# VatsalPandey0202/PointCloudRegistration

Measured on AMD Instinct MI355X. Metric: TOF/PC pairs/sec (8192 pts), higher is better.
Workload: dtype f32 xyz/features; f64 RANSAC/ICP; 1-term f16 MFMA screen (certified bound), f16x3-split MFMA screen for the rows it leaves, f64 exact re-rank; 1 GPU; C4: batch of augmented TOF/PC pairs (featNN+RANSAC+ICP+Chamfer); pairs_total=256, pairs_per_gpu=256, points=8192, feature_dim=32, streams_per_gpu=1, ransac=d=0.04 mutual n=3 edge0.9 dist0.04 (100000,0.999), icp=d=0.02 (1e-6,1e-6,30), parallelism=pair-sharded x1, inputs=resident in HBM (--full: host_resident is the PCIe-inclusive rate)

## Files before the change

pointcloudregistration_amd/csrc/featnn_thresh.h:

```cpp
#pragma once
#include <stdint.h>
#include <string.h>

#if defined(__HIPCC__)
#define PCR_THRESH_HD __host__ __device__
#else
#define PCR_THRESH_HD
#endif

namespace pcr {

PCR_THRESH_HD inline uint32_t thresh_bits_up(double t) {
    if (!(t == t)) return 0x7f800000u;
    if (!(t > 0.0)) return 0u;
    const float f = (float)t;
    uint32_t b;
    memcpy(&b, &f, sizeof(b));
    return (double)f < t ? b + 1u : b;
}

PCR_THRESH_HD inline int thresh_flush_count(uint32_t base, uint32_t local, int K) {
    if (base >= (uint32_t)K) return 0;
    const uint32_t room = (uint32_t)K - base;
    return (int)(local < room ? local : room);
}

}
```

pointcloudregistration_amd/csrc/featnn_thresh.hip:

```cpp
#include "featnn_v5.h"
#include "featnn_thresh.h"
#include <stdlib.h>
#include <algorithm>
#include <cstdio>
#include <type_traits>

namespace pcr {
namespace {

__device__ unsigned g_thresh_stat[2][3];

#ifndef PCR_THRESH_G
#define PCR_THRESH_G 16
#endif
#ifndef PCR_THRESH_PF
#define PCR_THRESH_PF 1
#endif
constexpr int kThreshG = PCR_THRESH_G;

__device__ __forceinline__ unsigned lds_add_rtn(unsigned addr, unsigned v) {
    unsigned r;
    asm volatile("ds_add_rtn_u32 %0, %1, %2\n\ts_waitcnt lgkmcnt(0)" : "=v"(r) : "v"(addr), "v"(v) : "memory");
    return r;
}
__device__ __forceinline__ void lds_store(unsigned addr, int v) {
    asm volatile("ds_write_b32 %0, %1\n\ts_waitcnt lgkmcnt(0)" : : "v"(addr), "v"(v) : "memory");
}

template <int S, bool kIdx>
__global__ __launch_bounds__(512) void featnn_thresh9(RowArgs5 a) {
    constexpr int NB = S, W = 8, RT = 2, G = kThreshG, GS = G / 2;
    constexpr int kT = G * NB * 64;
    constexpr int kRows = W * RT * 32;
    static_assert(G % 2 == 0 && kRows == 512, "whole steps; the flush is one row per thread");
    __shared__ __attribute__((aligned(16))) f16x8 Bs0[kT];
    __shared__ __attribute__((aligned(16))) f16x8 Bs1[kT];
    __shared__ __attribute__((aligned(16))) float Cs0[G * 32];
    __shared__ __attribute__((aligned(16))) float Cs1[G * 32];
    __shared__ unsigned hcnt[kRows];
    __shared__ int hslot[kRows * kThreshK];
    const int nbp = gridDim.x / (8 * ((a.P + 7) >> 3));
    const int bid = blockIdx.x, xcd = bid & 7, slot = bid >> 3;
    const int p = (slot / nbp) * 8 + xcd, sl = slot % nbp;
    if (p >= a.P) return;
    const int nr = min(a.rcount[p], a.Rmax);
    const int m = count_of(a.n_cols, p, a.Cmax);
    const int nst = (((m + 31) >> 5) + 1) >> 1;
    const int nsl = min(nbp, nst);
    if (nr <= 0 || sl >= nsl) return;
    const int s0 = (int)((long long)nst * sl / nsl), s1 = (int)((long long)nst * (sl + 1) / nsl);
    const int ngr = (s1 - s0 + GS - 1) / GS;
    const int wid = threadIdx.x >> 6, l = threadIdx.x & 63, h = l >> 5;
    const int ntl = (nr + 31) >> 5;
    const int *rl = a.rlist + (size_t)p * a.Rmax;
    const int nm = a.ich;
    const f16x8 *bimg = a.Bp + (size_t)p * a.ntc * nm * 64 + l;
    const float *ctp = a.cct + (size_t)p * a.ntc * 32 + l;
    auto issue = [&](auto bufc_, int grp) {
        f16x8 *Bs = decltype(bufc_)::value ? Bs1 : Bs0;
        float *Cs = decltype(bufc_)::value ? Cs1 : Cs0;
        const int sg = s0 + grp * GS;
        for (int c = wid; c < G * NB + GS; c += W) {
            if (c >= G * NB) {
                const int j = c - G * NB;
                if (sg + j < s1)
                    __builtin_amdgcn_global_load_lds(
                        (const __attribute__((address_space(1))) void *)(ctp + (size_t)(sg + j) * 64),
                        (__attribute__((address_space(3))) void *)(Cs + j * 64),
                        4, 0, 0);
                continue;
            }
            const int g = c / NB, cc = c - g * NB;
            if (sg + (g >> 1) < s1)
                __builtin_amdgcn_global_load_lds(
                    (const __attribute__((address_space(1))) void *)(bimg + ((size_t)(2 * sg + g) * nm + cc) * 64),
                    (__attribute__((address_space(3))) void *)(Bs + c * 64), 16, 0, 0);
        }
    };
    auto min8 = [](const f32x16 &x, int q) {
        unsigned c = umin2(umin2(fbits(x[8 * q]), fbits(x[8 * q + 1])), fbits(x[8 * q + 2]));
        c = umin2(umin2(c, fbits(x[8 * q + 3])), fbits(x[8 * q + 4]));
        c = umin2(umin2(c, fbits(x[8 * q + 5])), fbits(x[8 * q + 6]));
        return umin2(c, fbits(x[8 * q + 7]));
    };
    for (int tb = 0; tb < ntl; tb += W * RT) {
        hcnt[threadIdx.x] = 0u;
        issue(std::integral_constant<int, 0>{}, 0);
        const int nt = tb + wid + W < ntl ? 2 : (tb + wid < ntl ? 1 : 0);
        size_t o[RT];
        unsigned B1[RT], thr[RT], am[RT];
        bool live[RT];
        int nh[RT], lr[RT];
        unsigned ca[RT], sa[RT];
        f16x8 A[RT][NB];
#pragma unroll
        for (int t = 0; t < RT; ++t) {
            lr[t] = (t * W + wid) * 32 + (l & 31);
            ca[t] = (unsigned)(uintptr_t)(hcnt + lr[t]);
            sa[t] = (unsigned)(uintptr_t)(hslot + lr[t] * kThreshK);
            const int k = tb * 32 + lr[t];
            const bool valid = k < nr;
            const int row = valid ? rl[k] : 0;
            o[t] = (size_t)p * a.Rmax + row;
            B1[t] = valid ? a.rec[o[t]].y : 0x7f800000u;
            thr[t] = 0u;
            live[t] = false;
            if (valid && B1[t] < 0x7f800000u) {
                const double bnd = row_bound_ct(a, p, row, a.rre[(size_t)p * a.ntr * 32 + row], 16 * S);
                thr[t] = thresh_bits_up((double)__uint_as_float(B1[t]) + bnd * (1.0 + 0x1p-20));
                live[t] = thr[t] < 0x7f800000u;
            }
            row_operand<S, 3>(a, p, row, valid, h, A[t]);
            am[t] = 0xffffffffu;
            nh[t] = 0;
        }
        auto sweep = [&](auto ntc_, auto bufc_, int grp) {
            constexpr int NT = decltype(ntc_)::value;
            const f16x8 *Bs = decltype(bufc_)::value ? Bs1 : Bs0;
            const float *Cb = decltype(bufc_)::value ? Cs1 : Cs0;
            const int sg = s0 + grp * GS, ns = min(GS, s1 - sg);
            const f16x8 *Bb = Bs + l;
            auto load = [&](int j, f16x8 (&Bf)[2][NB], f32x16 (&Cf)[2]) {
#pragma unroll
                for (int u = 0; u < 2; ++u) {
#pragma unroll
                    for (int c = 0; c < NB; ++c) Bf[u][c] = Bb[((2 * j + u) * NB + c) * 64];
                    Cf[u] = colterms(Cb + (2 * j + u) * 32, h);
                }
            };
            f16x8 Bf[2][NB];
            f32x16 Cf[2];
            if (PCR_THRESH_PF) load(0, Bf, Cf);
            for (int j = 0; j < ns; ++j) {
                const int st = sg + j;
                f16x8 Bn[2][NB];
                f32x16 Cn[2];
                if (PCR_THRESH_PF) load(j + 1 < ns ? j + 1 : j, Bn, Cn);
                else load(j, Bf, Cf);
                f32x16 acc[NT][2];
#pragma unroll
                for (int c = 0; c < NB; ++c)
#pragma unroll
                    for (int u = 0; u < 2; ++u)
#pragma unroll
                        for (int t = 0; t < NT; ++t)
                            acc[t][u] = __builtin_amdgcn_mfma_f32_32x32x16_f16(Bf[u][c], A[t][c],
                                                                               c == 0 ? Cf[u] : acc[t][u], 0, 0, 0);
#pragma unroll
                for (int t = 0; t < NT; ++t)
#pragma unroll
                    for (int u = 0; u < 2; ++u) {
                        const unsigned m0 = min8(acc[t][u], 0), m1 = min8(acc[t][u], 1);
                        if (__ballot(umin2(m0, m1) <= thr[t]) == 0ull) continue;
                        const bool half[2] = {__ballot(m0 <= thr[t]) != 0ull, __ballot(m1 <= thr[t]) != 0ull};
#pragma unroll
                        for (int r = 0; r < 16; ++r) {
                            if (!half[r >> 3]) continue;
                            const unsigned v = fbits(acc[t][u][r]);
                            const int col = 32 * (2 * st + u) + 8 * (r >> 2) + 4 * h + (r & 3);
                            if (v <= thr[t] && live[t] && col < m) {
                                if (kIdx && v == B1[t]) am[t] = umin2(am[t], (unsigned)col);
                                if (nh[t] <= kThreshK) {
                                    const unsigned pos = lds_add_rtn(ca[t], 1u);
                                    if (pos < (unsigned)kThreshK) lds_store(sa[t] + 4u * pos, col);
                                }
                                ++nh[t];
                            }
                        }
                    }
                if (PCR_THRESH_PF) {
#pragma unroll
                    for (int u = 0; u < 2; ++u) {
#pragma unroll
                        for (int c = 0; c < NB; ++c) Bf[u][c] = Bn[u][c];
                        Cf[u] = Cn[u];
                    }
                }
            }
        };
        asm volatile("s_waitcnt vmcnt(0)" ::: "memory");
        __syncthreads();
        auto group = [&](auto bufc_, int grp) {
            constexpr int buf = decltype(bufc_)::value;
            if (grp + 1 < ngr) issue(std::integral_constant<int, buf ^ 1>{}, grp + 1);
            if (nt == 2) sweep(std::integral_constant<int, 2>{}, bufc_, grp);
            else if (nt == 1) sweep(std::integral_constant<int, 1>{}, bufc_, grp);
            asm volatile("s_waitcnt vmcnt(0)" ::: "memory");
            __syncthreads();
        };
        for (int grp = 0; grp < ngr; grp += 2) {
            group(std::integral_constant<int, 0>{}, grp);
            if (grp + 1 < ngr) group(std::integral_constant<int, 1>{}, grp + 1);
        }
#pragma unroll
        for (int t = 0; t < RT; ++t)
            if (kIdx && am[t] != 0xffffffffu) atomicMin(reinterpret_cast<unsigned *>(a.rec + o[t]) + 2, am[t]);
        {
            const int r = threadIdx.x, k = tb * 32 + r;
            const unsigned lc = hcnt[r];
            if (k < nr && lc != 0u) {
                const size_t oo = (size_t)p * a.Rmax + rl[k];
                const unsigned base = atomicAdd(reinterpret_cast<unsigned *>(a.rec + oo), lc);
                const int n = thresh_flush_count(base, lc, kThreshK);
                for (int i = 0; i < n; ++i) a.cand[oo * kThreshK + base + i] = hslot[r * kThreshK + i];
            }
        }
        __syncthreads();
    }
}

template <int DV, bool kIdx>
__global__ __launch_bounds__(256) void featnn_exact_cand(RowArgs5 a) {
    const int p = blockIdx.y;
    const int nr = min(a.rcount[p], a.Rmax);
    if (nr <= 0) return;
    if (blockIdx.x == 0 && threadIdx.x == 0) atomicAdd(a.fbctr + (kIdx ? 0 : 1), (unsigned long long)nr);
    const int m = count_of(a.n_cols, p, a.Cmax);
    const int *rl = a.rlist + (size_t)p * a.Rmax;
    const int c = threadIdx.x & 7, rr = threadIdx.x >> 3, D = a.D;
    const float4 open = make_float4(__builtin_inff(), __builtin_inff(), __builtin_inff(), 0.0f);
    for (int k0 = blockIdx.x * 32; k0 < nr; k0 += gridDim.x * 32) {
        const bool act = k0 + rr < nr;
        const int row = act ? rl[k0 + rr] : 0;
        const size_t o = (size_t)p * a.Rmax + row;
        const uint4 rc = act ? a.rec[o] : make_uint4(0u, 0x7f800000u, 0u, 1u);
        const int cnt = (int)min(rc.x, (unsigned)kThreshK + 1u);
        double best = __builtin_inf();
        int bj = 0x7fffffff;
        if (act && m > 0 && c < cnt && cnt <= kThreshK && rc.y < 0x7f800000u) {
            const int j = a.cand[o * kThreshK + c];
            const float *q = a.Xr + o * D, *y = a.Xc + ((size_t)p * a.Cmax + j) * D;
            float qf[DV], yf[DV];
            if (D == DV && (((uintptr_t)q | (uintptr_t)y) & 15) == 0) {
#pragma unroll
                for (int k = 0; k < DV; k += 4) {
                    const float4 u = *reinterpret_cast<const float4 *>(q + k), w = *reinterpret_cast<const float4 *>(y + k);
                    qf[k] = u.x; qf[k + 1] = u.y; qf[k + 2] = u.z; qf[k + 3] = u.w;
                    yf[k] = w.x; yf[k + 1] = w.y; yf[k + 2] = w.z; yf[k + 3] = w.w;
                }
            } else {
#pragma unroll
                for (int k = 0; k < DV; ++k) {
                    qf[k] = k < D ? q[k] : 0.0f;
                    yf[k] = k < D ? y[k] : 0.0f;
                }
            }
            double acc = 0.0;
#pragma unroll
            for (int k = 0; k < DV; ++k) {
                const double df = (double)qf[k] - (double)yf[k];
                acc = acc + df * df;
            }
            if (acc < best) { best = acc; bj = j; }
        }
#pragma unroll
        for (int x = 1; x < 8; x <<= 1) {
            const double ob = __shfl_xor(best, x, 64);
// ... 86 lines not shown
```

pointcloudregistration_amd/csrc/featnn_row.hip:

```cpp
#include "featnn_v5.h"
#include <stdlib.h>
#include <algorithm>

namespace pcr {
namespace {

__device__ unsigned long long g_featnn_fallback_rows[2];

template <int S>
__device__ __forceinline__ void row_frags(const float *x, int D, int h, int role, int cs,
                                          f16x8 (&out)[2 * S + 1]) {
    constexpr int DV = 16 * S;
    double acc = 0.0;
#pragma unroll
    for (int k = 0; k < DV; ++k)
        if (k < D) {
            const double v = (double)x[k];
            acc = acc + v * v;
        }
    _Float16 np[3];
    double wv = acc * __builtin_ldexp(1.0, -cs);
#pragma unroll
    for (int q = 0; q < 3; ++q) {
        np[q] = (_Float16)(float)wv;
        wv = wv - (double)np[q];
    }
    const _Float16 cval = (_Float16)__builtin_ldexpf(1.0f, cs);
    _Float16 s0[DV], s1[DV];
#pragma unroll
    for (int k = 0; k < DV; ++k) {
        const _Float16 hi = (_Float16)x[k];
        const _Float16 lo = (_Float16)(x[k] - (float)hi);
        s0[k] = role == 0 ? (_Float16)(-2.0f * (float)hi) : hi;
        s1[k] = role == 0 ? (_Float16)(-2.0f * (float)lo) : lo;
    }
#pragma unroll
    for (int c = 0; c < 2 * S + 1; ++c) {
#pragma unroll
        for (int j = 0; j < 8; ++j) {
            _Float16 v0 = (_Float16)0.0f, v1 = (_Float16)0.0f;
            if (c < 2 * S) {
                const int k0 = 16 * (c % S) + j;
                const _Float16 *sg = c < S ? s0 : s1;
                v0 = k0 < D ? sg[k0] : (_Float16)0.0f;
                v1 = k0 + 8 < D ? sg[k0 + 8] : (_Float16)0.0f;
            } else {
                if (j < 3) v0 = role == 0 ? np[j] : cval;
                else if (j < 6) v0 = role == 0 ? cval : np[j - 3];
                else if (j == 6 && role == 1) v0 = (_Float16)32768.0f;
                else if (j == 7 && role == 0) v0 = (_Float16)32768.0f;
            }
            out[c][j] = h ? v1 : v0;
        }
    }
// ... 490 lines not shown
            B2 = umin2(umin2(B2, o2), umax2(B1, o1));
            const bool take = o1 < B1;
            B1 = take ? o1 : B1;
            jw = take ? oj : jw;
        }
        const int mi1 = (int)(B1 & ctmask) * 32 + jw;
        const int k = qt * 32 + R;
        if (h != 0 || k >= nr) continue;
        const int row = rl ? rl[k] : k;
        if (csl > 1) {
            a.part[((size_t)p * csl + sl) * a.Rmax + k] = make_uint4(B1, B2, (unsigned)mi1, 0u);
            continue;
        }
        if (row_tail<kIdx, kOne, NX>(a, p, row, m, B1, B2, mi1, rex[t], __builtin_ldexp(1.0, a.ctbits - 23)))
            a.list[(size_t)p * a.Rmax + atomicAdd(a.count + p, 1)] = row;
    }
}

template <int S, bool kIdx>
__global__ __launch_bounds__(256) void featnn_slicemerge(RowArgs5 a) {
    constexpr int NX = 3 * S + 1;
    const int p = blockIdx.y, k = blockIdx.x * 256 + threadIdx.x;
    const int *rl = a.rlist + (size_t)p * a.Rmax;
    if (k >= a.rcount[p]) return;
    unsigned B1 = 0x7f800000u, B2 = 0x7f800000u, mi = 0u;
    for (int s2 = 0; s2 < a.csl; ++s2) {
        const uint4 q = a.part[((size_t)p * a.csl + s2) * a.Rmax + k];
        B2 = umin2(umin2(B2, q.y), umax2(B1, q.x));
        mi = q.x < B1 ? q.z : mi;
        B1 = umin2(B1, q.x);
    }
    const int row = rl[k];
    if (row_tail<kIdx, false, NX>(a, p, row, count_of(a.n_cols, p, a.Cmax), B1, B2, (int)mi, 0.0f,
                                  __builtin_ldexp(1.0, a.ctbits - 23)))
        a.list[(size_t)p * a.Rmax + atomicAdd(a.count + p, 1)] = row;
}


__device__ __forceinline__ unsigned group_min32(const f32x16 &x, const f32x16 &y) {
    unsigned c0 = umin2(umin2(fbits(x[0]), fbits(x[1])), fbits(x[2]));
    unsigned c1 = umin2(umin2(fbits(x[11]), fbits(x[12])), fbits(x[13]));
    unsigned c2 = umin2(umin2(fbits(y[6]), fbits(y[7])), fbits(y[8]));
#pragma unroll
    for (int r = 3; r < 11; r += 2) c0 = umin2(umin2(c0, fbits(x[r])), fbits(x[r + 1]));
    c1 = umin2(umin2(c1, fbits(x[14])), fbits(x[15]));
#pragma unroll
    for (int r = 0; r < 6; r += 2) c1 = umin2(umin2(c1, fbits(y[r])), fbits(y[r + 1]));
#pragma unroll
    for (int r = 9; r < 15; r += 2) c2 = umin2(umin2(c2, fbits(y[r])), fbits(y[r + 1]));
    c2 = umin2(c2, fbits(y[15]));
    return umin2(umin2(c0, c1), c2);
}

template <int S, int G, bool kIdx>
__global__ __launch_bounds__(512) __attribute__((amdgpu_waves_per_eu(4))) void featnn_row9(RowArgs5 a) {
    constexpr int W = 8, RT = 2;
    constexpr int NB = S;
    constexpr int kT = G * NB * 64;
    constexpr int kB = kT + G * 8;
    static_assert(G % 8 == 0 && S <= 2, "column tiles in pairs; the terms in whole 1 KB DMA pieces");
    constexpr int kTC = G / 8;
    __shared__ __attribute__((aligned(16))) f16x8 Bs[2 * kB];
    const int b = blockIdx.x, xcd = b & 7, slot = b >> 3;
    const int ppx = (a.P + 7) >> 3;
    const int p = a.rbmajor ? (slot % ppx) * 8 + xcd : (slot / a.nrb) * 8 + xcd;
    const int rb = a.rbmajor ? slot / ppx : slot - (slot / a.nrb) * a.nrb;
    if (p >= a.P) return;
    const int *rl = a.rlist ? a.rlist + (size_t)p * a.Rmax : nullptr;
    const int nr = rl ? a.rcount[p] : count_of(a.n_rows, p, a.Rmax);
    if (rb * W * RT * 32 >= nr) return;
    const int wid = threadIdx.x >> 6, l = threadIdx.x & 63, h = l >> 5;
    const int m = count_of(a.n_cols, p, a.Cmax);
    const int qt0 = (rb * W + wid) * RT;
    const int ntc = (m + 31) >> 5;
    const int ngroups = (ntc + G - 1) / G;
    f16x8 A[RT][NB];
#pragma unroll
    for (int t = 0; t < RT; ++t) {
        const int k = (qt0 + t) * 32 + (l & 31);
        row_operand<S, kIdx ? 0 : 1>(a, p, rl ? (k < nr ? rl[k] : 0) : (k < nr ? k : 0), k < nr, h, A[t]);
    }
    unsigned B1[RT], B2[RT], I[RT], pm[RT];
#pragma unroll
    for (int t = 0; t < RT; ++t) { B1[t] = 0x7f800000u; B2[t] = 0x7f800000u; I[t] = 0u; pm[t] = 0x7f800000u; }
    const int nm = a.ich;
    const f16x8 *bsrc = a.Bp + (size_t)p * a.ntc * nm * 64 + l;
    const float *csrc = a.cct + (size_t)p * a.ntc * 32 + 4 * l;
    auto issue = [&](int grp, int bufi) {
        for (int c = wid; c < G * NB + kTC; c += W) {
            if (c >= G * NB) {
                const int tc = c - G * NB;
                __builtin_amdgcn_global_load_lds(
                    (const __attribute__((address_space(1))) void *)(csrc + (size_t)grp * G * 32 + tc * 256),
                    (__attribute__((address_space(3))) void *)(Bs + bufi * kB + kT + tc * 64), 16, 0, 0);
                continue;
            }
            const int g = c / NB, cc = c - g * NB;
            const f16x8 *src = bsrc + ((size_t)(grp * G + g) * nm + cc) * 64;
            __builtin_amdgcn_global_load_lds(
                (const __attribute__((address_space(1))) void *)src,
                (__attribute__((address_space(3))) void *)(Bs + bufi * kB + c * 64), 16, 0, 0);
        }
    };
    auto min16 = [](const f32x16 &x, unsigned c0) {
        unsigned c1 = umin2(umin2(fbits(x[8]), fbits(x[9])), fbits(x[10]));
        c0 = umin2(umin2(c0, fbits(x[0])), fbits(x[1]));
        c1 = umin2(umin2(c1, fbits(x[11])), fbits(x[12]));
        c0 = umin2(umin2(c0, fbits(x[2])), fbits(x[3]));
// ... 54 lines not shown
#pragma unroll
        for (int c = 0; c < NB; ++c) Bf[c] = Bb[c * 64];
        Cf = cnext(0);
        __builtin_amdgcn_sched_barrier(0);
#pragma unroll
        for (int st = 0; st < G / 2; ++st) {
            const unsigned stp = (unsigned)(grp * (G / 2) + st);
#pragma unroll
            for (int c = 0; c < NB; ++c)
#pragma unroll
                for (int t = 0; t < RT; ++t)
                    acc[t][0] = __builtin_amdgcn_mfma_f32_32x32x16_f16(Bf[c], A[t][c], c == 0 ? Cf : acc[t][0], 0, 0, 0);
#pragma unroll
            for (int t = 0; t < RT; ++t) close(acc[t][1], t, pend);
#pragma unroll
            for (int c = 0; c < NB; ++c) Bf[c] = Bb[((2 * st + 1) * NB + c) * 64];
            Cf = cnext(2 * st + 1);
            SGB(0x002, 2, 0);
#pragma unroll
            for (int i = 0; i < NB * RT; ++i) {
                SGB(0x008, 1, 0);
                SGB(0x002, 5, 0);
            }
            SGB(0x100, NB + kCR, 0);
            SGB(0x002, 6 + kCV, 0);
            __builtin_amdgcn_sched_barrier(0);
#pragma unroll
            for (int c = 0; c < NB; ++c)
#pragma unroll
                for (int t = 0; t < RT; ++t)
                    acc[t][1] = __builtin_amdgcn_mfma_f32_32x32x16_f16(Bf[c], A[t][c], c == 0 ? Cf : acc[t][1], 0, 0, 0);
#pragma unroll
            for (int t = 0; t < RT; ++t) pm[t] = min16(acc[t][0], 0x7f800000u);
            if (st + 1 < G / 2) {
#pragma unroll
                for (int c = 0; c < NB; ++c) Bf[c] = Bb[((2 * st + 2) * NB + c) * 64];
                Cf = cnext(2 * st + 2);
            }
#pragma unroll
            for (int i = 0; i < NB * RT; ++i) {
                SGB(0x008, 1, 0);
                SGB(0x002, 4, 0);
            }
            if (st + 1 < G / 2) SGB(0x100, NB + kCR, 0);
            if (st + 1 < G / 2 && kCV) SGB(0x002, kCV, 0);
            __builtin_amdgcn_sched_barrier(0);
            pend = stp;
        }
        asm volatile("s_waitcnt vmcnt(0)" ::: "memory");
        __syncthreads();
    }
#pragma unroll
    for (int t = 0; t < RT; ++t) close(acc[t][1], t, pend);
    const int nst = a.ntc >> 1;
#pragma unroll
    for (int t = 0; t < RT; ++t) {
        const unsigned o1 = (unsigned)__shfl_xor((int)B1[t], 32, 64);
        const unsigned o2 = (unsigned)__shfl_xor((int)B2[t], 32, 64);
        const unsigned oi = (unsigned)__shfl_xor((int)I[t], 32, 64);
        const unsigned s2 = umin2(umax2(B1[t], o1), umin2(B2[t], o2));
        const bool mine = B1[t] < o1 || (B1[t] == o1 && h == 0);
        const unsigned w1 = mine ? B1[t] : o1;
        const unsigned wst = min(mine ? I[t] : oi, (unsigned)(nst - 1));
        const int k = (qt0 + t) * 32 + (l & 31);
        if (h == 0 && k < nr) {
            const int row = rl ? reinterpret_cast<const volatile int *>(rl)[k] : k;
            const size_t bk = (size_t)p * nst + wst;
            const bool early = one_term_fails<kIdx, S>(a, p, row, w1, s2, a.rre[(size_t)p * a.ntr * 32 + row],
                                                       a.rct[(size_t)p * a.ntr * 32 + row]);
            const int rank = early ? a.bcap : atomicAdd(a.bcnt + bk, 1);
            if (rank < a.bcap) {
                a.blist[bk * a.bcap + rank] = make_uint4((unsigned)row, w1, s2, mine ? 0u : 1u);
            } else {
                a.rec[(size_t)p * a.Rmax + row] = make_uint4(0u, w1, 0xffffffffu, 1u);
                a.list[(size_t)p * a.Rmax + atomicAdd(a.count + p, 1)] = row;
            }
        }
    }
}

template <int S, bool kIdx>
__global__ __launch_bounds__(256) __attribute__((amdgpu_waves_per_eu(4))) void featnn_regroup9(RowArgs5 a) {
    constexpr int NB = S;
    extern __shared__ int rg_lds[];
    __shared__ int wsum[4];
    const int nst = a.ntc >> 1;
    int *ts = rg_lds, *cn = rg_lds + nst + 1;
    const int nbp = gridDim.x / (8 * ((a.P + 7) >> 3));
    const int bid = blockIdx.x, xcd = bid & 7, slot = bid >> 3;
    const int p = (slot / nbp) * 8 + xcd, bx = slot % nbp;
    if (p >= a.P) return;
    const int t = threadIdx.x, wid = t >> 6, l = t & 63, h = l >> 5;
    const int *bc = a.bcnt + (size_t)p * nst;
    const int seg = (nst + 3) >> 2, s0 = min(nst, wid * seg), s1 = min(nst, s0 + seg);
    int run = 0;
    for (int c0 = s0; c0 < s1; c0 += 64) {
        const int i = c0 + l;
        const int ci = i < s1 ? min(bc[i], a.bcap) : 0;
        const int ti = (ci + 31) >> 5;
        int x = ti;
#pragma unroll
        for (int o = 1; o < 64; o <<= 1) {
            const int y = __shfl_up(x, o, 64);
            if (l >= o) x += y;
        }
        if (i < s1) {
            ts[i] = run + x - ti;
            cn[i] = ci;
        }
        run += __shfl(x, 63, 64);
    }
    if (l == 0) wsum[wid] = run;
    __syncthreads();
    int add = 0;
    for (int ww = 0; ww < wid; ++ww) add += wsum[ww];
    for (int i = s0 + l; i < s1; i += 64) ts[i] += add;
    if (t == 0) ts[nst] = wsum[0] + wsum[1] + wsum[2] + wsum[3];
    __syncthreads();
    const int ntiles = ts[nst];
    const int nm = a.ich;
    const f16x8 *bimg = a.Bp + (size_t)p * a.ntc * nm * 64 + l;
    const float *ctp = a.cct + (size_t)p * a.ntc * 32;
    const uint4 *bl = a.blist + (size_t)p * nst * a.bcap;
    auto locate = [&](int q, int &b, bool &valid, uint4 &e) {
        int lo = 0, hi = nst;
        while (hi - lo > 1) {
            const int md = (lo + hi) >> 1;
            if (ts[md] <= q) lo = md;
            else hi = md;
        }
        b = lo;
// ... 87 lines not shown
    __syncthreads();
    if (t == 0) {
        const int tot = wcnt[0] + wcnt[1] + wcnt[2] + wcnt[3];
        base = tot && a.llist ? atomicAdd(a.lcount + p, tot) : 0;
    }
    __syncthreads();
    if (!a.llist) return;
    int off = base + x - mine;
    for (int ww = 0; ww < w; ++ww) off += wcnt[ww];
#pragma unroll
    for (int i = 0; i < R; ++i)
        if (put[i]) a.llist[(size_t)p * a.Rmax + off++] = rows[i];
}

}

constexpr int kRow7RT = 1, kRow7G = 4;

template <bool kIdx>
int launch_row7(const RowArgs5 &r0, int S, hipStream_t s) {
    RowArgs5 r = r0;
    PCR_REQUIRE(r.ich == 2 * S + 1, PCR_ERR_ARG, "featnn_row7: needs the full operand image (%d chunks)", r.ich);
    r.nrb = cdiv(cdiv(r.Rmax, 32), 8 * kRow7RT);
    const long long nblk = 8LL * r.nrb * cdiv(r.P, 8);
    PCR_REQUIRE(nblk < (1LL << 31), PCR_ERR_ARG, "feature_match: grid too large");
    const dim3 grid((unsigned)nblk);
    if (S == 3) hipLaunchKernelGGL((featnn_row7<3, kRow7G, kIdx, kRow7RT>), grid, dim3(512), 0, s, r);
    else if (S == 4) hipLaunchKernelGGL((featnn_row7<4, kRow7G, kIdx, kRow7RT>), grid, dim3(512), 0, s, r);
    else { set_error("feature dim too large for the f16 split screen"); return PCR_ERR_ARG; }
    PCR_LAUNCH_CHECK();
    return PCR_OK;
}

template <bool kIdx, bool kOne>
int launch_row8(const RowArgs5 &r0, int S, hipStream_t s) {
    RowArgs5 r = r0;
    PCR_REQUIRE(r.ich == 2 * S + 1, PCR_ERR_ARG, "featnn_row8: needs the full operand image (%d chunks)", r.ich);
    r.nrb = cdiv(cdiv(r.Rmax, 32), 8 * 2);
    const int csl = r.rbmajor ? r.csl : 1;
    const long long nblk = 8LL * r.nrb * csl * cdiv(r.P, 8);
    PCR_REQUIRE(nblk < (1LL << 31), PCR_ERR_ARG, "feature_corres: grid too large");
    if (S == 1) hipLaunchKernelGGL((featnn_row8<1, kRow8G, kIdx, kOne>), dim3((unsigned)nblk), dim3(512), 0, s, r);
    else hipLaunchKernelGGL((featnn_row8<2, kRow8G, kIdx, kOne>), dim3((unsigned)nblk), dim3(512), 0, s, r);
    PCR_LAUNCH_CHECK();
    if (csl > 1) {
        const dim3 mg(cdiv(r.Rmax, 256), r.P);
        if (S == 1) hipLaunchKernelGGL((featnn_slicemerge<1, kIdx>), mg, dim3(256), 0, s, r);
        else hipLaunchKernelGGL((featnn_slicemerge<2, kIdx>), mg, dim3(256), 0, s, r);
        PCR_LAUNCH_CHECK();
    }
    return PCR_OK;
}

template <bool kIdx>
int launch_row9(const RowArgs5 &r0, int S, hipStream_t s) {
    RowArgs5 r = r0;
    PCR_REQUIRE(r.ich == S || r.ich == 2 * S + 1, PCR_ERR_ARG, "featnn_row9: image of %d chunks per tile", r.ich);
    r.nrb = cdiv(cdiv(r.Rmax, 32), 8 * 2);
    const long long nblk = 8LL * r.nrb * cdiv(r.P, 8);
    PCR_REQUIRE(nblk < (1LL << 31), PCR_ERR_ARG, "feature_corres: grid too large");
    constexpr int G = kIdx ? kRow9G1 : kRow9G;
    if (S == 1) hipLaunchKernelGGL((featnn_row9<1, G, kIdx>), dim3((unsigned)nblk), dim3(512), 0, s, r);
    else hipLaunchKernelGGL((featnn_row9<2, G, kIdx>), dim3((unsigned)nblk), dim3(512), 0, s, r);
    PCR_LAUNCH_CHECK();
    return PCR_OK;
}

template <bool kIdx>
int launch_regroup9(const RowArgs5 &r, int S, hipStream_t s) {
    static const int tpb = [] {
        const char *e = getenv("PCR_REGROUP_TPB");
        const int v = e ? atoi(e) : 24;
        return v >= 4 ? v : 24;
    }();
    const int nbp = cdiv(cdiv(r.Rmax, 32) + r.ntc / 2, tpb);
    const dim3 grid((unsigned)(8LL * nbp * cdiv(r.P, 8)));
    const dim3 fgrid(cdiv(r.Rmax, 1024), r.P);
    const size_t sm = sizeof(int) * (2 * (size_t)(r.ntc / 2) + 1);
    if (S == 1) {
        hipLaunchKernelGGL((featnn_regroup9<1, kIdx>), grid, dim3(256), sm, s, r);
        hipLaunchKernelGGL((featnn_finish9<1, kIdx>), fgrid, dim3(256), 0, s, r);
    } else {
        hipLaunchKernelGGL((featnn_regroup9<2, kIdx>), grid, dim3(256), sm, s, r);
        hipLaunchKernelGGL((featnn_finish9<2, kIdx>), fgrid, dim3(256), 0, s, r);
    }
    PCR_LAUNCH_CHECK();
    return PCR_OK;
}

int fallback_counter(unsigned long long **ctr) {
    PCR_HIP_CHECK(hipGetSymbolAddress((void **)ctr, HIP_SYMBOL(g_featnn_fallback_rows)));
    return PCR_OK;
}

template int launch_row7<true>(const RowArgs5 &, int, hipStream_t);
template int launch_row7<false>(const RowArgs5 &, int, hipStream_t);
template int launch_row8<true, true>(const RowArgs5 &, int, hipStream_t);
template int launch_row8<true, false>(const RowArgs5 &, int, hipStream_t);
template int launch_row8<false, true>(const RowArgs5 &, int, hipStream_t);
template int launch_row8<false, false>(const RowArgs5 &, int, hipStream_t);
template int launch_row9<true>(const RowArgs5 &, int, hipStream_t);
template int launch_row9<false>(const RowArgs5 &, int, hipStream_t);
template int launch_regroup9<true>(const RowArgs5 &, int, hipStream_t);
template int launch_regroup9<false>(const RowArgs5 &, int, hipStream_t);

}

extern "C" int pcr_featnn_fallback_rows(int64_t *rows12, int64_t *cols21, int32_t reset) {
    pcr::clear_error();
    unsigned long long v[2] = {0, 0};
    PCR_HIP_CHECK(hipDeviceSynchronize());
    PCR_HIP_CHECK(hipMemcpyFromSymbol(v, HIP_SYMBOL(pcr::g_featnn_fallback_rows), sizeof(v)));
    if (rows12) *rows12 = (int64_t)v[0];
    if (cols21) *cols21 = (int64_t)v[1];
    if (reset) {
        const unsigned long long z[2] = {0, 0};
// ... 5 lines not shown
```

Before: 51200 pairs/s.

## Balance threshold screen work across waves via flattened tile-step items with LDS row operands

Row operands and per-row metadata (threshold, best value, flags, argmin) are staged in LDS so any wave can process any row tile. The tile×step work is then split evenly across the 8 waves instead of each wave owning fixed tiles, which removes idle waves when the last row block is partial. Hit recording now uses ds_min and LDS flag bits with no per-store waitcnt, and the default B/C prefetch is turned off. The cost is extra LDS traffic and footprint for A operands each step, with possibly lower occupancy.

Measured after the change: 51600 pairs/s, median of 6. Within noise of the previous version (+0.8%).

```diff
diff --git a/pointcloudregistration_amd/csrc/featnn_thresh.h b/pointcloudregistration_amd/csrc/featnn_thresh.h
--- a/pointcloudregistration_amd/csrc/featnn_thresh.h
+++ b/pointcloudregistration_amd/csrc/featnn_thresh.h
@@ -25,4 +25,17 @@
     return (int)(local < room ? local : room);
 }
 
+PCR_THRESH_HD inline void thresh_item_range(int ntiles, int nsteps, int wave, int nwaves, int *begin, int *end) {
+    const int n = ntiles > 0 && nsteps > 0 ? ntiles * nsteps : 0;
+    *begin = (int)((long long)n * wave / nwaves);
+    *end = (int)((long long)n * (wave + 1) / nwaves);
 }
+
+PCR_THRESH_HD inline void thresh_item_run(int ntiles, int i, int end, int *step, int *t0, int *t1) {
+    *step = i / ntiles;
+    *t0 = i - *step * ntiles;
+    const int left = end - i;
+    *t1 = *t0 + left < ntiles ? *t0 + left : ntiles;
+}
+
+}
diff --git a/pointcloudregistration_amd/csrc/featnn_thresh.hip b/pointcloudregistration_amd/csrc/featnn_thresh.hip
--- a/pointcloudregistration_amd/csrc/featnn_thresh.hip
+++ b/pointcloudregistration_amd/csrc/featnn_thresh.hip
@@ -14,7 +14,7 @@
 #define PCR_THRESH_G 16
 #endif
 #ifndef PCR_THRESH_PF
-#define PCR_THRESH_PF 1
+#define PCR_THRESH_PF 0
 #endif
 constexpr int kThreshG = PCR_THRESH_G;
 
@@ -24,8 +24,12 @@
     return r;
 }
 __device__ __forceinline__ void lds_store(unsigned addr, int v) {
-    asm volatile("ds_write_b32 %0, %1\n\ts_waitcnt lgkmcnt(0)" : : "v"(addr), "v"(v) : "memory");
-}
+    asm volatile("ds_write_b32 %0, %1" : : "v"(addr), "v"(v) : "memory");
+}
+__device__ __forceinline__ void lds_min(unsigned addr, unsigned v) {
+    asm volatile("ds_min_u32 %0, %1" : : "v"(addr), "v"(v) : "memory");
+}
+__device__ __forceinline__ void lds_drain() { asm volatile("s_waitcnt vmcnt(0) lgkmcnt(0)" ::: "memory"); }
 
 template <int S, bool kIdx>
 __global__ __launch_bounds__(512) void featnn_thresh9(RowArgs5 a) {
@@ -39,6 +43,8 @@
     __shared__ __attribute__((aligned(16))) float Cs1[G * 32];
     __shared__ unsigned hcnt[kRows];
     __shared__ int hslot[kRows * kThreshK];
+    __shared__ __attribute__((aligned(16))) f16x8 As[W * RT * NB * 64];
+    __shared__ __attribute__((aligned(16))) uint4 rmeta[kRows];
     const int nbp = gridDim.x / (8 * ((a.P + 7) >> 3));
     const int bid = blockIdx.x, xcd = bid & 7, slot = bid >> 3;
     const int p = (slot / nbp) * 8 + xcd, sl = slot % nbp;
@@ -83,126 +89,165 @@
         c = umin2(umin2(c, fbits(x[8 * q + 5])), fbits(x[8 * q + 6]));
         return umin2(c, fbits(x[8 * q + 7]));
     };
+    const unsigned hcnt0 = (unsigned)(uintptr_t)hcnt, hslot0 = (unsigned)(uintptr_t)hslot;
+    const unsigned rmeta0 = (unsigned)(uintptr_t)rmeta;
     for (int tb = 0; tb < ntl; tb += W * RT) {
         hcnt[threadIdx.x] = 0u;
         issue(std::integral_constant<int, 0>{}, 0);
-        const int nt = tb + wid + W < ntl ? 2 : (tb + wid < ntl ? 1 : 0);
-        size_t o[RT];
-        unsigned B1[RT], thr[RT], am[RT];
-        bool live[RT];
-        int nh[RT], lr[RT];
-        unsigned ca[RT], sa[RT];
-        f16x8 A[RT][NB];
+        const int T = min(W * RT, ntl - tb);
 #pragma unroll
         for (int t = 0; t < RT; ++t) {
-            lr[t] = (t * W + wid) * 32 + (l & 31);
-            ca[t] = (unsigned)(uintptr_t)(hcnt + lr[t]);
-            sa[t] = (unsigned)(uintptr_t)(hslot + lr[t] * kThreshK);
-            const int k = tb * 32 + lr[t];
+            const int tile = t * W + wid;
+            if (tile >= T) continue;
+            const int lr = tile * 32 + (l & 31);
+            const int k = tb * 32 + lr;
             const bool valid = k < nr;
             const int row = valid ? rl[k] : 0;
-            o[t] = (size_t)p * a.Rmax + row;
-            B1[t] = valid ? a.rec[o[t]].y : 0x7f800000u;
-            thr[t] = 0u;
-            live[t] = false;
-            if (valid && B1[t] < 0x7f800000u) {
+            const size_t o = (size_t)p * a.Rmax + row;
+            const unsigned B1 = valid ? a.rec[o].y : 0x7f800000u;
+            unsigned thr = 0u;
+            bool live = false;
+            if (valid && B1 < 0x7f800000u) {
                 const double bnd = row_bound_ct(a, p, row, a.rre[(size_t)p * a.ntr * 32 + row], 16 * S);
-                thr[t] = thresh_bits_up((double)__uint_as_float(B1[t]) + bnd * (1.0 + 0x1p-20));
-                live[t] = thr[t] < 0x7f800000u;
-            }
-            row_operand<S, 3>(a, p, row, valid, h, A[t]);
-            am[t] = 0xffffffffu;
-            nh[t] = 0;
-        }
-        auto sweep = [&](auto ntc_, auto bufc_, int grp) {
-            constexpr int NT = decltype(ntc_)::value;
+                thr = thresh_bits_up((double)__uint_as_float(B1) + bnd * (1.0 + 0x1p-20));
+                live = thr < 0x7f800000u;
+            }
+            f16x8 A[NB];
+            row_operand<S, 3>(a, p, row, valid, h, A);
+#pragma unroll
+            for (int c = 0; c < NB; ++c) As[(tile * NB + c) * 64 + l] = A[c];
+            if (h == 0) rmeta[lr] = make_uint4(thr, B1, live ? 3u : 0u, 0xffffffffu);
+        }
+        auto sweep = [&](auto bufc_, int grp) {
             const f16x8 *Bs = decltype(bufc_)::value ? Bs1 : Bs0;
             const float *Cb = decltype(bufc_)::value ? Cs1 : Cs0;
             const int sg = s0 + grp * GS, ns = min(GS, s1 - sg);
-            const f16x8 *Bb = Bs + l;
-            auto load = [&](int j, f16x8 (&Bf)[2][NB], f32x16 (&Cf)[2]) {
-#pragma unroll
-                for (int u = 0; u < 2; ++u) {
-#pragma unroll
-                    for (int c = 0; c < NB; ++c) Bf[u][c] = Bb[((2 * j + u) * NB + c) * 64];
-                    Cf[u] = colterms(Cb + (2 * j + u) * 32, h);
+            const f16x8 *Bb = Bs + l, *Ab = As + l;
+            const uint4 *rb = rmeta + (l & 31);
+            auto loadA = [&](int t, int t1, f16x8 (&Af)[2][NB], uint4 (&rm)[2]) {
+#pragma unroll
+                for (int x = 0; x < 2; ++x) {
+                    const int tt = min(t + x, t1 - 1);
+#pragma unroll
+                    for (int c = 0; c < NB; ++c) Af[x][c] = Ab[(tt * NB + c) * 64];
+                    rm[x] = rb[tt * 32];
                 }
             };
-            f16x8 Bf[2][NB];
-            f32x16 Cf[2];
-            if (PCR_THRESH_PF) load(0, Bf, Cf);
-            for (int j = 0; j < ns; ++j) {
-                const int st = sg + j;
-                f16x8 Bn[2][NB];
-                f32x16 Cn[2];
-                if (PCR_THRESH_PF) load(j + 1 < ns ? j + 1 : j, Bn, Cn);
-                else load(j, Bf, Cf);
+            auto run = [&](auto ntc_, int t, int st, const f16x8 (&Bf)[2][NB], const f32x16 (&Cf)[2],
+                           const f16x8 (&Af)[2][NB], const uint4 (&rm)[2]) {
+                constexpr int NT = decltype(ntc_)::value;
                 f32x16 acc[NT][2];
 #pragma unroll
                 for (int c = 0; c < NB; ++c)
 #pragma unroll
                     for (int u = 0; u < 2; ++u)
 #pragma unroll
-                        for (int t = 0; t < NT; ++t)
-                            acc[t][u] = __builtin_amdgcn_mfma_f32_32x32x16_f16(Bf[u][c], A[t][c],
-                                                                               c == 0 ? Cf[u] : acc[t][u], 0, 0, 0);
-#pragma unroll
-                for (int t = 0; t < NT; ++t)
+                        for (int x = 0; x < NT; ++x)
+                            acc[x][u] = __builtin_amdgcn_mfma_f32_32x32x16_f16(Bf[u][c], Af[x][c],
+                                                                               c == 0 ? Cf[u] : acc[x][u], 0, 0, 0);
+#pragma unroll
+                for (int x = 0; x < NT; ++x) {
+                    const unsigned thr = rm[x].x, B1 = rm[x].y;
+                    unsigned fl = rm[x].z;
+                    const unsigned lr = (unsigned)((t + x) * 32 + (l & 31));
 #pragma unroll
                     for (int u = 0; u < 2; ++u) {
-                        const unsigned m0 = min8(acc[t][u], 0), m1 = min8(acc[t][u], 1);
-                        if (__ballot(umin2(m0, m1) <= thr[t]) == 0ull) continue;
-                        const bool half[2] = {__ballot(m0 <= thr[t]) != 0ull, __ballot(m1 <= thr[t]) != 0ull};
-#pragma unroll
-                        for (int r = 0; r < 16; ++r) {
-                            if (!half[r >> 3]) continue;
-                            const unsigned v = fbits(acc[t][u][r]);
-                            const int col = 32 * (2 * st + u) + 8 * (r >> 2) + 4 * h + (r & 3);
-                            if (v <= thr[t] && live[t] && col < m) {
-                                if (kIdx && v == B1[t]) am[t] = umin2(am[t], (unsigned)col);
-                                if (nh[t] <= kThreshK) {
-                                    const unsigned pos = lds_add_rtn(ca[t], 1u);
-                                    if (pos < (unsigned)kThreshK) lds_store(sa[t] + 4u * pos, col);
+                        const unsigned m0 = min8(acc[x][u], 0), m1 = min8(acc[x][u], 1);
+                        if (__ballot(umin2(m0, m1) <= thr) == 0ull) continue;
+                        const bool half[2] = {__ballot(m0 <= thr) != 0ull, __ballot(m1 <= thr) != 0ull};
+                        unsigned hm = 0u, em = 0u;
+#pragma unroll
+                        for (int q = 0; q < 2; ++q) {
+                            if (!half[q]) continue;
+#pragma unroll
+                            for (int r = 8 * q; r < 8 * q + 8; ++r) {
+                                const unsigned v = fbits(acc[x][u][r]);
+                                hm |= (v <= thr ? 1u : 0u) << r;
+                                if (kIdx) em |= (v == B1 ? 1u : 0u) << r;
+                            }
+                        }
+                        if (!(fl & 1u)) hm = 0u;
+                        const int cb = 32 * (2 * st + u) + 4 * h;
+                        while (hm != 0u) {
+                            const int r = __builtin_ctz(hm);
+                            hm &= hm - 1u;
+                            const int col = cb + 8 * (r >> 2) + (r & 3);
+                            if (col >= m) continue;
+                            if (kIdx && ((em >> r) & 1u)) lds_min(rmeta0 + 16u * lr + 12u, (unsigned)col);
+                            if (fl & 2u) {
+                                const unsigned pos = lds_add_rtn(hcnt0 + 4u * lr, 1u);
+                                if (pos < (unsigned)kThreshK) {
+                                    lds_store(hslot0 + 4u * (lr * kThreshK + pos), col);
+                                } else {
+                                    lds_store(rmeta0 + 16u * lr + 8u, 1);
+                                    fl = 1u;
                                 }
-                                ++nh[t];
                             }
                         }
                     }
-                if (PCR_THRESH_PF) {
-#pragma unroll
-                    for (int u = 0; u < 2; ++u) {
-#pragma unroll
-                        for (int c = 0; c < NB; ++c) Bf[u][c] = Bn[u][c];
-                        Cf[u] = Cn[u];
+                }
+            };
+            int ib, ie;
+            thresh_item_range(T, ns, wid, W, &ib, &ie);
+            for (int i = ib; i < ie;) {
+                int j, t0, t1;
+                thresh_item_run(T, i, ie, &j, &t0, &t1);
+                f16x8 Bf[2][NB];
+                f32x16 Cf[2];
+#pragma unroll
+                for (int u = 0; u < 2; ++u) {
+#pragma unroll
+                    for (int c = 0; c < NB; ++c) Bf[u][c] = Bb[((2 * j + u) * NB + c) * 64];
+                    Cf[u] = colterms(Cb + (2 * j + u) * 32, h);
+                }
+                f16x8 An[2][NB];
+                uint4 rn[2];
+                if (PCR_THRESH_PF) loadA(t0, t1, An, rn);
+                for (int t = t0; t < t1; t += 2) {
+                    f16x8 Af[2][NB];
+                    uint4 rm[2];
+                    if (PCR_THRESH_PF) {
+#pragma unroll
+                        for (int x = 0; x < 2; ++x) {
+#pragma unroll
+                            for (int c = 0; c < NB; ++c) Af[x][c] = An[x][c];
+                            rm[x] = rn[x];
+                        }
+                        if (t + 2 < t1) loadA(t + 2, t1, An, rn);
+                    } else {
+                        loadA(t, t1, Af, rm);
                     }
-                }
+                    if (t + 1 < t1) run(std::integral_constant<int, 2>{}, t, sg + j, Bf, Cf, Af, rm);
+                    else run(std::integral_constant<int, 1>{}, t, sg + j, Bf, Cf, Af, rm);
+                }
+                i += t1 - t0;
             }
         };
-        asm volatile("s_waitcnt vmcnt(0)" ::: "memory");
+        lds_drain();
         __syncthreads();
         auto group = [&](auto bufc_, int grp) {
             constexpr int buf = decltype(bufc_)::value;
             if (grp + 1 < ngr) issue(std::integral_constant<int, buf ^ 1>{}, grp + 1);
-            if (nt == 2) sweep(std::integral_constant<int, 2>{}, bufc_, grp);
-            else if (nt == 1) sweep(std::integral_constant<int, 1>{}, bufc_, grp);
-            asm volatile("s_waitcnt vmcnt(0)" ::: "memory");
+            sweep(bufc_, grp);
+            lds_drain();
             __syncthreads();
         };
         for (int grp = 0; grp < ngr; grp += 2) {
             group(std::integral_constant<int, 0>{}, grp);
             if (grp + 1 < ngr) group(std::integral_constant<int, 1>{}, grp + 1);
         }
-#pragma unroll
-        for (int t = 0; t < RT; ++t)
-            if (kIdx && am[t] != 0xffffffffu) atomicMin(reinterpret_cast<unsigned *>(a.rec + o[t]) + 2, am[t]);
         {
             const int r = threadIdx.x, k = tb * 32 + r;
             const unsigned lc = hcnt[r];
-            if (k < nr && lc != 0u) {
+            if (k < nr && r < T * 32) {
                 const size_t oo = (size_t)p * a.Rmax + rl[k];
-                const unsigned base = atomicAdd(reinterpret_cast<unsigned *>(a.rec + oo), lc);
-                const int n = thresh_flush_count(base, lc, kThreshK);
-                for (int i = 0; i < n; ++i) a.cand[oo * kThreshK + base + i] = hslot[r * kThreshK + i];
+                const unsigned am = rmeta[r].w;
+                if (kIdx && am != 0xffffffffu) atomicMin(reinterpret_cast<unsigned *>(a.rec + oo) + 2, am);
+                if (lc != 0u) {
+                    const unsigned base = atomicAdd(reinterpret_cast<unsigned *>(a.rec + oo), lc);
+                    const int n = thresh_flush_count(base, lc, kThreshK);
+                    for (int i = 0; i < n; ++i) a.cand[oo * kThreshK + base + i] = hslot[r * kThreshK + i];
+                }
             }
         }
         __syncthreads();
```

## Add column-sharded row9 screen that keeps row operands in LDS and merges across waves

Applied to the files above, without the earlier changes.

Adds a new form of the featnn_row9 screen kernel. Each block stages 16 row tiles of A in LDS, and its waves split the column steps among themselves, streaming B directly from global memory. The per-wave best and second-best results are then merged through LDS before the existing settle logic runs. This form becomes the default for both index modes, with a 256-thread, 4-wave variant selected unless an environment variable overrides it. The aim is more reuse of each loaded B tile across many row tiles and less LDS staging of B, at the cost of an extra cross-wave merge and a different occupancy profile.

Result: faster. 51900 pairs/s before, 53650 pairs/s after, median of 6 (+3.4%).

```diff
diff --git a/pointcloudregistration_amd/csrc/featnn_row.hip b/pointcloudregistration_amd/csrc/featnn_row.hip
--- a/pointcloudregistration_amd/csrc/featnn_row.hip
+++ b/pointcloudregistration_amd/csrc/featnn_row.hip
@@ -1,5 +1,7 @@
 #include "featnn_v5.h"
+#include "row9_merge.h"
 #include <stdlib.h>
+#include <string.h>
 #include <algorithm>
 
 namespace pcr {
@@ -596,8 +598,34 @@
     return umin2(umin2(c0, c1), c2);
 }
 
+template <int S, bool kIdx>
+__device__ __forceinline__ void row9_settle(const RowArgs5 &a, int p, const int *rl, int nr, int k, int h,
+                                            unsigned B1, unsigned B2, unsigned I) {
+    const int nst = a.ntc >> 1;
+    const unsigned o1 = (unsigned)__shfl_xor((int)B1, 32, 64);
+    const unsigned o2 = (unsigned)__shfl_xor((int)B2, 32, 64);
+    const unsigned oi = (unsigned)__shfl_xor((int)I, 32, 64);
+    const unsigned s2 = umin2(umax2(B1, o1), umin2(B2, o2));
+    const bool mine = B1 < o1 || (B1 == o1 && h == 0);
+    const unsigned w1 = mine ? B1 : o1;
+    const unsigned wst = min(mine ? I : oi, (unsigned)(nst - 1));
+    if (h == 0 && k < nr) {
+        const int row = rl ? reinterpret_cast<const volatile int *>(rl)[k] : k;
+        const size_t bk = (size_t)p * nst + wst;
+        const bool early = one_term_fails<kIdx, S>(a, p, row, w1, s2, a.rre[(size_t)p * a.ntr * 32 + row],
+                                                   a.rct[(size_t)p * a.ntr * 32 + row]);
+        const int rank = early ? a.bcap : atomicAdd(a.bcnt + bk, 1);
+        if (rank < a.bcap) {
+            a.blist[bk * a.bcap + rank] = make_uint4((unsigned)row, w1, s2, mine ? 0u : 1u);
+        } else {
+            a.rec[(size_t)p * a.Rmax + row] = make_uint4(0u, w1, 0xffffffffu, 1u);
+            a.list[(size_t)p * a.Rmax + atomicAdd(a.count + p, 1)] = row;
+        }
+    }
+}
+
 template <int S, int G, bool kIdx>
-__global__ __launch_bounds__(512) __attribute__((amdgpu_waves_per_eu(4))) void featnn_row9(RowArgs5 a) {
+__device__ __forceinline__ void row9_rows(const RowArgs5 &a) {
     constexpr int W = 8, RT = 2;
     constexpr int NB = S;
     constexpr int kT = G * NB * 64;
@@ -758,31 +786,138 @@
     }
 #pragma unroll
     for (int t = 0; t < RT; ++t) close(acc[t][1], t, pend);
-    const int nst = a.ntc >> 1;
+#pragma unroll
+    for (int t = 0; t < RT; ++t)
+        row9_settle<S, kIdx>(a, p, rl, nr, (qt0 + t) * 32 + (l & 31), h, B1[t], B2[t], I[t]);
+}
+
+template <int S, int G, bool kIdx, int W>
+__device__ __forceinline__ void row9_cols(const RowArgs5 &a) {
+    constexpr int NT = 16, RT = NT / W;
+    constexpr int NB = S;
+    constexpr int kOp = NT * NB * 64;
+    constexpr int kMg = W * W * 3 * 16;
+    static_assert(G % 2 == 0 && NT % W == 0 && S <= 2, "column tiles in pairs; whole row tiles per wave");
+    __shared__ __attribute__((aligned(16))) f16x8 As[kOp > kMg ? kOp : kMg];
+    const int b = blockIdx.x, xcd = b & 7, slot = b >> 3;
+    const int ppx = (a.P + 7) >> 3;
+    const int p = a.rbmajor ? (slot % ppx) * 8 + xcd : (slot / a.nrb) * 8 + xcd;
+    const int rb = a.rbmajor ? slot / ppx : slot - (slot / a.nrb) * a.nrb;
+    if (p >= a.P) return;
+    const int *rl = a.rlist ? a.rlist + (size_t)p * a.Rmax : nullptr;
+    const int nr = rl ? a.rcount[p] : count_of(a.n_rows, p, a.Rmax);
+    if (rb * NT * 32 >= nr) return;
+    const int wid = __builtin_amdgcn_readfirstlane(threadIdx.x >> 6), l = threadIdx.x & 63, h = l >> 5;
+    const int m = count_of(a.n_cols, p, a.Cmax);
+    const int ntc = (m + 31) >> 5;
+    const int nsteps = (ntc + G - 1) / G * (G / 2);
+    f16x8 *Asl = As + l;
 #pragma unroll
     for (int t = 0; t < RT; ++t) {
-        const unsigned o1 = (unsigned)__shfl_xor((int)B1[t], 32, 64);
-        const unsigned o2 = (unsigned)__shfl_xor((int)B2[t], 32, 64);
-        const unsigned oi = (unsigned)__shfl_xor((int)I[t], 32, 64);
-        const unsigned s2 = umin2(umax2(B1[t], o1), umin2(B2[t], o2));
-        const bool mine = B1[t] < o1 || (B1[t] == o1 && h == 0);
-        const unsigned w1 = mine ? B1[t] : o1;
-        const unsigned wst = min(mine ? I[t] : oi, (unsigned)(nst - 1));
-        const int k = (qt0 + t) * 32 + (l & 31);
-        if (h == 0 && k < nr) {
-            const int row = rl ? reinterpret_cast<const volatile int *>(rl)[k] : k;
-            const size_t bk = (size_t)p * nst + wst;
-            const bool early = one_term_fails<kIdx, S>(a, p, row, w1, s2, a.rre[(size_t)p * a.ntr * 32 + row],
-                                                       a.rct[(size_t)p * a.ntr * 32 + row]);
-            const int rank = early ? a.bcap : atomicAdd(a.bcnt + bk, 1);
-            if (rank < a.bcap) {
-                a.blist[bk * a.bcap + rank] = make_uint4((unsigned)row, w1, s2, mine ? 0u : 1u);
-            } else {
-                a.rec[(size_t)p * a.Rmax + row] = make_uint4(0u, w1, 0xffffffffu, 1u);
-                a.list[(size_t)p * a.Rmax + atomicAdd(a.count + p, 1)] = row;
-            }
-        }
-    }
+        const int tt = wid * RT + t;
+        const int k = (rb * NT + tt) * 32 + (l & 31);
+        f16x8 A[NB];
+        row_operand<S, kIdx ? 0 : 1>(a, p, rl ? (k < nr ? rl[k] : 0) : (k < nr ? k : 0), k < nr, h, A);
+#pragma unroll
+        for (int c = 0; c < NB; ++c) Asl[(tt * NB + c) * 64] = A[c];
+    }
+    __syncthreads();
+    unsigned B1[NT], B2[NT], I[NT];
+#pragma unroll
+    for (int t = 0; t < NT; ++t) { B1[t] = kRow9Inf; B2[t] = kRow9Inf; I[t] = 0u; }
+    const int nm = a.ich;
+    const f16x8 *bsrc = a.Bp + (size_t)p * a.ntc * nm * 64 + l;
+    const int *csrc = reinterpret_cast<const int *>(a.cct + (size_t)p * a.ntc * 32) + 8 * ((l & 15) >> 2) + (l & 3) + 4 * h;
+    auto load = [&](int st, f16x8 (&Bf)[2][NB], int (&cv)[2]) {
+#pragma unroll
+        for (int u = 0; u < 2; ++u) {
+#pragma unroll
+            for (int c = 0; c < NB; ++c) Bf[u][c] = bsrc[((size_t)(2 * st + u) * nm + c) * 64];
+            cv[u] = csrc[(2 * st + u) * 32];
+        }
+    };
+    auto cterms = [](f32x16 &c, int v) {
+#define PCR_BC(r) c[r] = __int_as_float(__builtin_amdgcn_mov_dpp(v, 0x150 + (r), 0xf, 0xf, false))
+        PCR_BC(0); PCR_BC(1); PCR_BC(2); PCR_BC(3); PCR_BC(4); PCR_BC(5); PCR_BC(6); PCR_BC(7);
+        PCR_BC(8); PCR_BC(9); PCR_BC(10); PCR_BC(11); PCR_BC(12); PCR_BC(13); PCR_BC(14); PCR_BC(15);
+#undef PCR_BC
+    };
+    f16x8 Bf[2][NB], Ar[2][NB];
+    int cv[2];
+    f32x16 acc[2][2];
+    if (wid < nsteps) {
+        load(wid, Bf, cv);
+#pragma unroll
+        for (int c = 0; c < NB; ++c) Ar[0][c] = Asl[c * 64];
+    }
+    for (int st = wid; st < nsteps; st += W) {
+        f32x16 Cf[2];
+        cterms(Cf[0], cv[0]);
+        cterms(Cf[1], cv[1]);
+        f16x8 Bn[2][NB];
+        int cn[2];
+        load(st + W < nsteps ? st + W : st, Bn, cn);
+        __builtin_amdgcn_sched_barrier(0);
+#pragma unroll
+        for (int t = 0; t < NT; ++t) {
+            const int cur = t & 1;
+#pragma unroll
+            for (int c = 0; c < NB; ++c)
+#pragma unroll
+                for (int u = 0; u < 2; ++u)
+                    acc[cur][u] = __builtin_amdgcn_mfma_f32_32x32x16_f16(Bf[u][c], Ar[cur][c],
+                                                                         c == 0 ? Cf[u] : acc[cur][u], 0, 0, 0);
+#pragma unroll
+            for (int c = 0; c < NB; ++c) Ar[cur ^ 1][c] = Asl[(((t + 1) % NT) * NB + c) * 64];
+            if (t > 0)
+                row9_close(B1[t - 1], B2[t - 1], I[t - 1], group_min32(acc[cur ^ 1][0], acc[cur ^ 1][1]), (unsigned)st);
+            SGB(0x008, 1, 0);
+            SGB(0x100, NB, 0);
+#pragma unroll
+            for (int i = 1; i < 2 * NB; ++i) {
+                SGB(0x002, 20 / (2 * NB), 0);
+                SGB(0x008, 1, 0);
+            }
+            __builtin_amdgcn_sched_barrier(0);
+        }
+        row9_close(B1[NT - 1], B2[NT - 1], I[NT - 1], group_min32(acc[1][0], acc[1][1]), (unsigned)st);
+#pragma unroll
+        for (int u = 0; u < 2; ++u) {
+#pragma unroll
+            for (int c = 0; c < NB; ++c) Bf[u][c] = Bn[u][c];
+            cv[u] = cn[u];
+        }
+    }
+    unsigned *mg = reinterpret_cast<unsigned *>(As) + l;
+    unsigned M1[RT], M2[RT], MI[RT];
+#pragma unroll
+    for (int r = 0; r < RT; ++r) {
+        __syncthreads();
+#pragma unroll
+        for (int j = 0; j < W; ++j) {
+            unsigned *q = mg + (wid * W + j) * 3 * 64;
+            q[0] = B1[RT * j + r];
+            q[64] = B2[RT * j + r];
+            q[128] = I[RT * j + r];
+        }
+        __syncthreads();
+        M1[r] = kRow9Inf; M2[r] = kRow9Inf; MI[r] = 0u;
+#pragma unroll
+        for (int w = 0; w < W; ++w) {
+            const unsigned *q = mg + (w * W + wid) * 3 * 64;
+            row9_merge(M1[r], M2[r], MI[r], q[0], q[64], q[128]);
+        }
+    }
+#pragma unroll
+    for (int r = 0; r < RT; ++r)
+        row9_settle<S, kIdx>(a, p, rl, nr, (rb * NT + wid * RT + r) * 32 + (l & 31), h, M1[r], M2[r], MI[r]);
+}
+
+template <int S, int G, int kForm, bool kIdx>
+__global__ __launch_bounds__(kForm == 1 ? 256 : 512) __attribute__((amdgpu_waves_per_eu(kForm ? 2 : 4)))
+void featnn_row9(RowArgs5 a) {
+    if constexpr (kForm == 0) row9_rows<S, G, kIdx>(a);
+    else row9_cols<S, G, kIdx, kForm == 1 ? 4 : 8>(a);
 }
 
 template <int S, bool kIdx>
@@ -976,6 +1111,14 @@
     return PCR_OK;
 }
 
+#ifndef PCR_ROW9_FORM1
+#define PCR_ROW9_FORM1 1
+#endif
+#ifndef PCR_ROW9_FORM2
+#define PCR_ROW9_FORM2 1
+#endif
+constexpr int kRow9Form1 = PCR_ROW9_FORM1, kRow9Form2 = PCR_ROW9_FORM2;
+
 template <bool kIdx>
 int launch_row9(const RowArgs5 &r0, int S, hipStream_t s) {
     RowArgs5 r = r0;
@@ -984,8 +1127,22 @@
     const long long nblk = 8LL * r.nrb * cdiv(r.P, 8);
     PCR_REQUIRE(nblk < (1LL << 31), PCR_ERR_ARG, "feature_corres: grid too large");
     constexpr int G = kIdx ? kRow9G1 : kRow9G;
-    if (S == 1) hipLaunchKernelGGL((featnn_row9<1, G, kIdx>), dim3((unsigned)nblk), dim3(512), 0, s, r);
-    else hipLaunchKernelGGL((featnn_row9<2, G, kIdx>), dim3((unsigned)nblk), dim3(512), 0, s, r);
+    int form = kIdx ? kRow9Form1 : kRow9Form2;
+    if (const char *e = getenv("PCR_ROW9_SWEEP")) {
+        if (!strcmp(e, "rows")) form = 0;
+        else if (!strcmp(e, "cols")) form = 1;
+        else if (!strcmp(e, "cols8")) form = 2;
+    }
+    const dim3 grid((unsigned)nblk);
+#define PCR_ROW9_LAUNCH(S_)                                                                                     \
+    do {                                                                                                        \
+        if (form == 0) hipLaunchKernelGGL((featnn_row9<S_, G, 0, kIdx>), grid, dim3(512), 0, s, r);             \
+        else if (form == 1) hipLaunchKernelGGL((featnn_row9<S_, G, 1, kIdx>), grid, dim3(256), 0, s, r);        \
+        else hipLaunchKernelGGL((featnn_row9<S_, G, 2, kIdx>), grid, dim3(512), 0, s, r);                       \
+    } while (0)
+    if (S == 1) PCR_ROW9_LAUNCH(1);
+    else PCR_ROW9_LAUNCH(2);
+#undef PCR_ROW9_LAUNCH
     PCR_LAUNCH_CHECK();
     return PCR_OK;
 }
diff --git a/pointcloudregistration_amd/csrc/row9_merge.h b/pointcloudregistration_amd/csrc/row9_merge.h
--- /dev/null
+++ b/pointcloudregistration_amd/csrc/row9_merge.h
@@ -0,0 +1,31 @@
+#pragma once
+
+#if defined(__HIPCC__) || defined(__CUDACC__)
+#define PCR_ROW9_HD __host__ __device__ __forceinline__
+#else
+#define PCR_ROW9_HD inline
+#endif
+
+namespace pcr {
+
+constexpr unsigned kRow9Inf = 0x7f800000u;
+
+PCR_ROW9_HD unsigned row9_min(unsigned a, unsigned b) { return a < b ? a : b; }
+PCR_ROW9_HD unsigned row9_max(unsigned a, unsigned b) { return a > b ? a : b; }
+
+PCR_ROW9_HD void row9_close(unsigned &b1, unsigned &b2, unsigned &i, unsigned mn, unsigned st) {
+    const unsigned n2 = row9_max(row9_min(b1, b2), row9_min(row9_max(b1, b2), mn));
+    i = mn < b1 ? st : i;
+    b1 = row9_min(b1, mn);
+    b2 = n2;
+}
+
+PCR_ROW9_HD void row9_merge(unsigned &b1, unsigned &b2, unsigned &i, unsigned o1, unsigned o2, unsigned oi) {
+    const unsigned n2 = row9_min(row9_max(b1, o1), row9_min(b2, o2));
+    const bool take = o1 < b1 || (o1 == b1 && oi < i);
+    i = take ? oi : i;
+    b1 = row9_min(b1, o1);
+    b2 = n2;
+}
+
+}
```
